# AugmentariumLab/VolumeRenderer

Hardware: AMD Instinct MI355X
Metric: Mvoxels/s kd-tree compress+decode (higher is better)
Workload: dtype u8; 1 GPU; 2048x2048x1920 uint8 volume per GPU as 960 bricks of 256x256x128, rm_volume, tolerance 1, maxEpochs 2, VolumeKdtree build + levelCut

## Files before the change

### volumerenderer_amd/csrc/kd_encode.hip

```cpp
#include "brickset.h"
#include <math.h>
#include <stdio.h>
#include <stdlib.h>
#include <string.h>

namespace vr {

#define FILL_NODES_PER_BLOCK 1024
#define EMIT_RANKS_PER_BLOCK 256

template <bool FROM_VOXELS>
__global__ void __launch_bounds__(256)
k_pyramid(Geom g, int dLeaf, int L, const uint8_t *__restrict__ vox, const uint8_t *__restrict__ inMin,
          const uint8_t *__restrict__ inMax, int64_t inStride, uint8_t *__restrict__ temp, int64_t heapStride,
          uint8_t *__restrict__ tempRange, uint8_t *__restrict__ outMin, uint8_t *__restrict__ outMax,
          int64_t outStride, const uint32_t *__restrict__ srcIdx)
{
    __shared__ uint8_t smn[2][1024], smx[2][1024];
    const int brick = blockIdx.y;
    const uint32_t n = 1u << L;
    const uint32_t base = blockIdx.x << L;
    uint8_t *T = temp + (int64_t)brick * heapStride;
    uint8_t *TR = tempRange ? tempRange + (int64_t)brick * heapStride : nullptr;
    for (uint32_t i = threadIdx.x; i < n; i += blockDim.x) {
// ... 210 lines not shown
    }
    const vr_s16x2 mn3 = pk_pair_min(pk_u(mn2[0]), pk_u(mn2[1])), mx3 = pk_pair_max(pk_u(mx2[0]), pk_u(mx2[1]));
    {
        const int64_t o = ((int64_t)1 << (D - 3)) + (base >> 3) + t * 2;
        const uint32_t m3 = pk_mid(mn3, mx3), h3 = pk_half_range(mn3, mx3);
        *(uint16_t *)(T + o) = (uint16_t)((m3 & 0xFFu) | ((m3 >> 8) & 0xFF00u));
        if (TR) *(uint16_t *)(TR + o) = (uint16_t)((h3 & 0xFFu) | ((h3 >> 8) & 0xFF00u));
    }
    int mn = min((int)mn3.x, (int)mn3.y), mx = max((int)mx3.x, (int)mx3.y);
    {
        const int64_t o = ((int64_t)1 << (D - 4)) + (base >> 4) + t;
        T[o] = (uint8_t)((mn + mx) >> 1);
        if (TR) TR[o] = (uint8_t)((mx - mn) >> 1);
    }
    uint32_t p = (uint32_t)mn | ((uint32_t)(255 - mx) << 16);
#pragma unroll
    for (int k = 1; k <= 6; ++k) {
        uint32_t q;
        if (k == 1) q = dpp_u32<0x101, 0xf>(p, p);
        else if (k == 2) q = dpp_u32<0x102, 0xf>(p, p);
        else if (k == 3) q = dpp_u32<0x104, 0xf>(p, p);
        else if (k == 4) q = dpp_u32<0x108, 0xf>(p, p);
        else q = (uint32_t)__shfl_down((int)p, 1 << (k - 1));
        p = pk_u(__builtin_elementwise_min(pk_s(p), pk_s(q)));
        if ((lane & ((1 << k) - 1)) == 0) {
            const int a = (int)(p & 0xFFFFu), b = 255 - (int)(p >> 16);
            const int64_t o = ((int64_t)1 << (D - 4 - k)) + (base >> (4 + k)) + (t >> k);
            T[o] = (uint8_t)((a + b) >> 1);
            if (TR) TR[o] = (uint8_t)((b - a) >> 1);
        }
    }
    if (lane == 0) mm[t >> 6] = p;
}

__device__ __forceinline__ void pyr12_box_root(const uint32_t *mm, int D, uint32_t base, int brick, uint8_t *__restrict__ T,
                                               uint8_t *__restrict__ TR, uint8_t *__restrict__ outMin, uint8_t *__restrict__ outMax,
                                               int64_t outStride, uint8_t *__restrict__ blockFlag, uint8_t *__restrict__ blockFlagR)
{
    {
        int a[2], b[2];
#pragma unroll
        for (int h = 0; h < 2; ++h) {
            const uint32_t u = pk_u(__builtin_elementwise_min(pk_s(mm[2 * h]), pk_s(mm[2 * h + 1])));
            a[h] = (int)(u & 0xFFFFu); b[h] = 255 - (int)(u >> 16);
            const int64_t o = ((int64_t)1 << (D - 11)) + (base >> 11) + h;
            T[o] = (uint8_t)((a[h] + b[h]) >> 1);
            if (TR) TR[o] = (uint8_t)((b[h] - a[h]) >> 1);
        }
        const int ra = min(a[0], a[1]), rbm = max(b[0], b[1]);
        const int64_t o = ((int64_t)1 << (D - 12)) + (base >> 12);
        T[o] = (uint8_t)((ra + rbm) >> 1);
        if (TR) TR[o] = (uint8_t)((rbm - ra) >> 1);
        outMin[(int64_t)brick * outStride + (base >> 12)] = (uint8_t)ra;
        outMax[(int64_t)brick * outStride + (base >> 12)] = (uint8_t)rbm;
        if (blockFlag) blockFlag[(int64_t)brick * ((int64_t)1 << (D - 12)) + (base >> 12)] = ra == rbm ? 1u : 0u;
        if (blockFlagR) blockFlagR[(int64_t)brick * ((int64_t)1 << (D - 12)) + (base >> 12)] = ra == rbm ? 1u : 0u;
    }
}

#ifndef VR_PYR_LINES_IMAGE_BOXES
#define VR_PYR_LINES_IMAGE_BOXES 8
#endif
#define PYR_LINES_IMAGE_STRIDE (4096 + 16)

__global__ void __launch_bounds__(256)
k_pyramid12_lines(Geom g, Pyr12Geom pg, const uint8_t *__restrict__ vox, uint8_t *__restrict__ temp, int64_t heapStride,
                  uint8_t *__restrict__ tempRange, uint8_t *__restrict__ outMin, uint8_t *__restrict__ outMax,
                  int64_t outStride, uint8_t *__restrict__ blockFlag, uint8_t *__restrict__ blockFlagR)
{
    constexpr int NB = VR_PYR_LINES_IMAGE_BOXES;
    static_assert(NB == 8 || NB == 4, "images per round");
    __shared__ __attribute__((aligned(16))) uint8_t leaf[NB * PYR_LINES_IMAGE_STRIDE];
    __shared__ uint32_t boxConst[4][8];
    __shared__ uint32_t waveMM[8][4];
    const int brick = blockIdx.y, D = g.D;
    const int t = threadIdx.x, lane = t & 63, c = t & 7;
    const uint32_t gid = blockIdx.x;
    const int lgx = pg.lnbx - 3;
    const int gx = (int)((gid & ((1u << lgx) - 1u)) << 7), by = (int)(((gid >> lgx) & ((1u << pg.lnby) - 1u)) << pg.ay),
              bz = (int)((gid >> (lgx + pg.lnby)) << pg.az);
    const int ymask = (1 << pg.ay) - 1;
    const uint8_t *src = vox + (int64_t)brick * g.voxels + (gx + c * 16) + (int64_t)g.X * (by + (int64_t)g.Y * bz);
    uint4 v[8];
#pragma unroll
    for (int k = 0; k < 8; ++k) {
        const int row = (t >> 3) + 32 * k;
        v[k] = *(const uint4 *)(src + (int64_t)g.X * ((row & ymask) + (int64_t)g.Y * (row >> pg.ay)));
    }
    const uint32_t *sp = pg.spread;
    const uint32_t rowBase = sp[g.X + by] | sp[g.X + g.Y + bz];
    uint8_t *T = temp + (int64_t)brick * heapStride;
    uint8_t *TR = tempRange ? tempRange + (int64_t)brick * heapStride : nullptr;
    uint32_t constMask = 0u;
    bool myConst = false;
    if (blockFlag) {
        const uint32_t v0 = __builtin_amdgcn_perm(0, v[0].x, 0u);
        uint32_t diff = 0u;
#pragma unroll
        for (int k = 0; k < 8; ++k) diff |= (v[k].x ^ v0) | (v[k].y ^ v0) | (v[k].z ^ v0) | (v[k].w ^ v0);
        const uint32_t ref = (uint32_t)__shfl((int)v0, c);
        const uint64_t same = __ballot(diff == 0u && v0 == ref), boxLanes = 0x0101010101010101ull << c;
        if (lane < 8) boxConst[t >> 6][lane] = (same & boxLanes) == boxLanes ? v0 : 0x100u;
        __syncthreads();
        const uint32_t c0 = boxConst[0][c];
        myConst = c0 != 0x100u && boxConst[1][c] == c0 && boxConst[2][c] == c0 && boxConst[3][c] == c0;
        constMask = (uint32_t)__ballot(myConst) & 0xFFu;
        if (constMask) {
            const int b = t >> 5, j = t & 31;
            const uint32_t cv = (uint32_t)__shfl((int)c0, b);
            if ((constMask >> b) & 1u) {
                const uint32_t base = sp[gx + 16 * b] | rowBase;
#pragma unroll
                for (int m = 0; m < 4; ++m)
                    pyr12_const_slot(j + 32 * m, cv, D, base, brick, T, TR, outMin, outMax, outStride, blockFlag, blockFlagR);
            }
            if (constMask == 0xFFu) return;
        }
    }
    const uint32_t rlo = sp[g.X + ((t >> 3) & ymask)] | sp[g.X + g.Y + ((t >> 3) >> pg.ay)];
    for (int h = 0; h < 8 / NB; ++h) {
        if (h) __syncthreads();
        if (!myConst && c / NB == h) {
            uint8_t *img = leaf + (c % NB) * PYR_LINES_IMAGE_STRIDE;
#pragma unroll
            for (int k = 0; k < 8; ++k) {
                const uint32_t r0 = rlo | sp[g.X + ((32 * k) & ymask)] | sp[g.X + g.Y + ((32 * k) >> pg.ay)];
                const uint32_t vw[4] = {v[k].x, v[k].y, v[k].z, v[k].w};
#pragma unroll
                for (int i = 0; i < 16; ++i) img[r0 | pg.sx[i]] = (uint8_t)(vw[i >> 2] >> ((i & 3) * 8));
            }
        }
        __syncthreads();
#pragma unroll 1
        for (int b = h * NB; b < (h + 1) * NB; ++b)
            if (!((constMask >> b) & 1u))
                pyr12_reduce_box(leaf + (b % NB) * PYR_LINES_IMAGE_STRIDE, D, sp[gx + 16 * b] | rowBase, t, T, TR, waveMM[b]);
    }
    __syncthreads();
    if (t < 8 && !((constMask >> t) & 1u))
        pyr12_box_root(waveMM[t], D, sp[gx + 16 * t] | rowBase, brick, T, TR, outMin, outMax, outStride, blockFlag, blockFlagR);
}

struct ReconBufs { uint8_t *b[3]; };

struct SkipBlocks {
    uint8_t *flag;
    int64_t nBlk;
    int Dm2;
};
__device__ __forceinline__ bool skip_block(const SkipBlocks &sk, int brick, int d, uint32_t node)
{
    return sk.flag && d > sk.Dm2 && (sk.flag[(int64_t)brick * sk.nBlk + (node >> (10 + d - sk.Dm2))] & 2u) != 0u;
}

__device__ inline int phys_buf(const Ctrl &c, int role) { return role == 0 ? c.ra : c.rb; }

__global__ void k_ctrl_init(Ctrl *ctrls, const uint8_t *rootMin, const uint8_t *rootMax, int64_t mmStride)
{
    Ctrl &c = ctrls[blockIdx.x];
    if (threadIdx.x) return;
    c.constBrick = 0; c.constVal = 0; c.zeroRun = 0;
    if (rootMin) {
        const int mn = rootMin[(int64_t)blockIdx.x * mmStride], mx = rootMax[(int64_t)blockIdx.x * mmStride];
        c.constBrick = mn == mx ? 1 : 0;
        c.constVal = mn;
    }
    c.currentDistance = c.currentError = c.currentDF = c.currentStepSize = 0.0;
    c.previousDistance = c.previousError = c.previousDF = c.previousStepSize = 0.0;
    c.errMinus = c.errPlus = 0;
    c.statL1 = 0;
    c.numActive = 0;
    c.epoch = 0; c.active = 0; c.fillThisEpoch = 0;
    c.cur = 0; c.prev = 1; c.pendingEqual = 0;
    c.par = 0; c.ra = 1; c.rb = 2;
    c.altValid = 0; c.altSel = 0; c.altDist = 0;
    c.numReverts = 0; c.maxErrBefore = 0; c.maxErrAfter = 0;
    c.estS = 0; c.estC = 0; c.estTbase = 0; c.estFallbacks = 0; c.estSeg = 0; c.estDone = 0; c.emitOverflow = 0;
    for (int i = 0; i < VR_MAX_DEPTH + 8; ++i) c.distanceMap[i] = 0;
}

#define EST_SEG 1024
#define EST_CAND 8
#define EST_ROUNDS 5
#define EST_HEAD 4096

#define est_at(ci, seg) (((int64_t)(ci) * summStride + (int64_t)(seg)) * 4)

__device__ __forceinline__ uint32_t wave_incl_scan_u32(uint32_t v, int lane)
{
    (void)lane;
    return wave_incl_scan_add_dpp(v);
}

__device__ __forceinline__ uint32_t lane_u32(uint32_t v, int l) { return (uint32_t)__builtin_amdgcn_readlane((int)v, l); }
__device__ __forceinline__ unsigned long long lane_u64(unsigned long long v, int l)
{
    return (unsigned long long)lane_u32((uint32_t)v, l) | ((unsigned long long)lane_u32((uint32_t)(v >> 32), l) << 32);
}

#define EST_STAGE_NODES 4096
__device__ inline void est_exact_chain(const uint8_t *__restrict__ T, const uint8_t *__restrict__ P, int d, uint32_t lo,
                                       uint32_t hi, unsigned long long &S, uint32_t &C, int lane, const SkipBlocks &sk, int brick,
                                       uint8_t *stage = nullptr)
{
    const uint32_t len = hi - lo;
    const bool staged = stage && d > 0 && len >= 64u && len <= (uint32_t)EST_STAGE_NODES && (len & 63u) == 0u && (lo & 31u) == 0u;
    const uint8_t *sT = stage, *sP = stage + EST_STAGE_NODES;
    if (staged) {
        for (uint32_t i = (uint32_t)lane * 16u; i < len; i += 1024u) *(uint4 *)(stage + i) = *(const uint4 *)(T + lo + i);
        for (uint32_t i = (uint32_t)lane * 16u; i < len / 2u; i += 1024u) *(uint4 *)(stage + EST_STAGE_NODES + i) = *(const uint4 *)(P + (lo >> 1) + i);
    }
    const bool sk0 = skip_block(sk, brick, d, lo);
    int tn = 0, pn = 0;
    if (staged) { tn = sT[lane]; pn = sP[lane >> 1]; }
    else { tn = (!sk0 && lo + lane < hi) ? T[lo + lane] : 0; pn = (!sk0 && lo + lane < hi && d > 0) ? P[(lo + lane) >> 1] : 0; }
    bool skipThis = sk0;
    for (uint32_t base = lo; base < hi; base += 64) {
        uint32_t i = base + lane;
        bool valid = i < hi;
        const int t = tn, p = pn;
        const bool skipped = skipThis;
        {
            const uint32_t i2 = i + 64;
            skipThis = base + 64 < hi && skip_block(sk, brick, d, base + 64);
            if (staged) {
                const uint32_t j2 = i2 - lo;
                tn = j2 < len ? sT[j2] : 0;
                pn = j2 < len ? sP[j2 >> 1] : 0;
            } else {
                tn = (!skipThis && i2 < hi) ? T[i2] : 0;
                pn = (!skipThis && i2 < hi && d > 0) ? P[i2 >> 1] : 0;
            }
        }
        if (skipped) continue;
        int pd = p > t ? p - t : t - p;
        bool forced = (t > p && 2 * t - p > 255) || (t < p && 2 * t < p);
        bool cand = valid && pd > 0;
        bool dec = cand && (forced || S < (unsigned long long)pd * (2ull * C + 1ull));
        unsigned long long mask = __ballot(dec);
        for (int it = 0; it < 65; ++it) {
            uint32_t cpre = __popcll(mask & ((1ull << lane) - 1ull));
            uint32_t v = dec ? (uint32_t)pd : 0u;
            uint32_t spre = wave_incl_scan_u32(v, lane) - v;
            bool nd = cand && (forced || (S + spre) < (unsigned long long)pd * (2ull * (C + cpre) + 1ull));
            unsigned long long nmask = __ballot(nd);
            dec = nd;
            if (nmask == mask) break;
            mask = nmask;
        }
        S += (uint32_t)__builtin_amdgcn_readlane((int)wave_incl_scan_add_dpp(dec ? (uint32_t)pd : 0u), 63);
        C += __popcll(mask);
    }
}

__device__ inline int est_window_base(long long T, int nc)
{
    long long b = T - (nc <= 4 ? 1 : 2);
    if (b < 0) b = 0;
    if (b > 256 - nc) b = 256 - nc;
    return (int)b;
}

__device__ inline void est_finish(Ctrl &c, unsigned long long S, uint32_t C, int maxEpochs)
{
    c.currentDistance = C > 0 ? round((double)S / (double)C) : 0.0;
    c.previousDistance = 0.0;
    c.previousStepSize = 255.0;
    c.previousError = 65025.0;
    c.epoch = 0;
    c.active = maxEpochs > 0 ? 1 : 0;
    c.fillThisEpoch = c.active;
    c.errMinus = c.errPlus = 0;
    c.cur = 0; c.prev = 1; c.pendingEqual = 0;
}

__global__ void __launch_bounds__(64)
k_est_head(int d, int maxEpochs, Ctrl *ctrls, const uint8_t *__restrict__ temp, int64_t heapStride, ReconBufs rb,
           int64_t leafStride, SkipBlocks sk)
{
    const int brick = blockIdx.x, lane = threadIdx.x;
    Ctrl &c = ctrls[brick];
    if (c.constBrick) return;
    const uint8_t *T = temp + (int64_t)brick * heapStride + ((int64_t)1 << d);
    const uint8_t *P = rb.b[c.par] + (int64_t)brick * leafStride;
    const uint32_t n = 1u << d;
    unsigned long long S = 0;
    uint32_t C = 0;
    __shared__ __attribute__((aligned(16))) uint8_t stage[EST_STAGE_NODES + EST_STAGE_NODES / 2];
    est_exact_chain(T, P, d, 0, n < EST_HEAD ? n : EST_HEAD, S, C, lane, sk, brick, stage);
    if (lane == 0) {
        if (n <= EST_HEAD) est_finish(c, S, C, maxEpochs);
        else {
            c.estS = S; c.estC = C;
            c.estSeg = EST_HEAD / EST_SEG;
            c.estDone = 0;
            c.estTbase = est_window_base((long long)(S / (2ull * C + 1ull)), 4);
        }
    }
}

__device__ __forceinline__ uint32_t seg_incl_scan_add_dpp(uint32_t v)
{
    v = row_incl_scan_add_dpp(v);
    return v + dpp_u32<0x142, 0xa>(0, v);
}
__device__ __forceinline__ int seg_max_i32_dpp(int v)
// ... 200 lines not shown
    uint32_t seg = (uint32_t)c.estSeg;
    int fallbacks = 0;
    uint32_t preSeg = 0xFFFFFFFFu;
    long long preCi = -1;
    uint4 pre[4];
#pragma unroll
    for (int j = 0; j < 4; ++j) pre[j] = make_uint4(0, 0, 0x80000000u, 0x7FFFFFFFu);
    const auto fetch = [&](long long ci_, uint32_t seg_, uint4 (&r)[4]) {
        const uint32_t k0 = seg_ + 4u * (uint32_t)lane;
#pragma unroll
        for (int j = 0; j < 4; ++j) {
            r[j] = make_uint4(0, 0, 0x80000000u, 0x7FFFFFFFu);
            if (k0 + (uint32_t)j < nseg) r[j] = *(const uint4 *)(sm + est_at((int)ci_, k0 + (uint32_t)j));
        }
    };
    while (seg < nseg) {
        const long long ci = Tc - Tbase;
        if (ci < 0 || ci >= nc || (budget >= 0 && !lastRound && fallbacks > budget)) {
            if (!lastRound) {
                if (lane == 0) {
                    c.estS = S; c.estC = C; c.estSeg = (int)seg;
                    c.estTbase = est_window_base(Tc, ncNext);
                    c.estFallbacks += fallbacks;
                }
                return;
            }
            est_exact_chain(T, P, d, seg * EST_SEG, n, S, C, lane, sk, brick);
            fallbacks += (int)(nseg - seg);
            break;
        }
        uint4 r[4];
        if (preSeg == seg && preCi == ci) {
#pragma unroll
            for (int j = 0; j < 4; ++j) r[j] = pre[j];
        } else fetch(ci, seg, r);
        preSeg = seg + 256u; preCi = ci;
        fetch(ci, preSeg, pre);
        const uint32_t k0 = seg + 4u * (uint32_t)lane;
        const uint32_t ssL = r[0].x + r[1].x + r[2].x + r[3].x, scL = r[0].y + r[1].y + r[2].y + r[3].y;
        const uint32_t si = wave_incl_scan_u32(ssL, lane), sci = wave_incl_scan_u32(scL, lane);
        uint32_t eS = si - ssL, eC = sci - scL;
        int failJ = 4;
        uint32_t fS = 0, fC = 0;
#pragma unroll
        for (int j = 0; j < 4; ++j) {
            const long long S0 = (long long)S + (long long)eS;
            const long long q = 2ll * ((long long)C + (long long)eC) + 1ll;
            const bool ok = k0 + (uint32_t)j >= nseg || (S0 - Tc * q >= (long long)(int)r[j].z && S0 - (Tc + 1) * q < (long long)(int)r[j].w);
            if (!ok && failJ == 4) { failJ = j; fS = eS; fC = eC; }
            eS += r[j].x; eC += r[j].y;
        }
        const unsigned long long bad = __ballot(failJ < 4);
        if (bad == 0ull) {
            S += lane_u32(si, 63);
            C += lane_u32(sci, 63);
            seg += 256u;
            continue;
        }
        const int f = __ffsll((long long)bad) - 1;
        S += lane_u32(fS, f);
        C += lane_u32(fC, f);
        seg += 4u * (uint32_t)f + lane_u32((uint32_t)failJ, f);
        est_exact_chain(T, P, d, seg * EST_SEG, (seg + 1) * EST_SEG, S, C, lane, sk, brick, stage);
        Tc = (long long)(S / (2ull * C + 1ull));
        seg += 1;
        ++fallbacks;
    }
    if (lane == 0) { est_finish(c, S, C, maxEpochs); c.estFallbacks += fallbacks; c.estDone = 1; }
}

__device__ inline unsigned long long block_sum_u64(unsigned long long v, unsigned long long *sh)
{
    for (int o = 32; o > 0; o >>= 1) v += __shfl_xor(v, o);
    const int w = threadIdx.x >> 6;
    if ((threadIdx.x & 63) == 0) sh[w] = v;
    __syncthreads();
    unsigned long long r = 0;
    if (threadIdx.x == 0) for (int i = 0; i < (int)(blockDim.x >> 6); ++i) r += sh[i];
    __syncthreads();
    return r;
}

__global__ void __launch_bounds__(256)
k_fill(int d, Ctrl *ctrls, const uint8_t *__restrict__ temp, uint8_t *__restrict__ codes, int64_t heapStride,
       int64_t codeStride, ReconBufs rb, int64_t leafStride, unsigned long long *__restrict__ blockErr, int64_t nErrBlk)
{
    __shared__ unsigned long long sh[4];
    const int brick = blockIdx.y;
    Ctrl &c = ctrls[brick];
    if (c.constBrick || !c.fillThisEpoch) return;
    const uint32_t n = 1u << d;
    const uint8_t *T = temp + (int64_t)brick * heapStride + ((int64_t)1 << d);
    uint8_t *Cb = codes + (int64_t)brick * codeStride;
    const uint8_t *P = rb.b[c.par] + (int64_t)brick * leafStride;
    uint8_t *R = rb.b[phys_buf(c, c.cur)] + (int64_t)brick * leafStride;
    const int dist = (int)(uint8_t)c.currentDistance;
    const int distM = (int)(uint8_t)fmax(0.0, c.currentDistance - 1.0);
    const int distP = (int)(uint8_t)fmin(255.0, c.currentDistance + 1.0);
    unsigned long long e0 = 0, em = 0, ep = 0;
    const uint32_t i0 = (blockIdx.x * 256u + threadIdx.x) * 4u;
    uint32_t pk = 0;
#pragma unroll
    for (int k = 0; k < 4; ++k) {
        uint32_t i = i0 + k;
        if (i < n) {
            int t = T[i];
            int p = d > 0 ? P[i >> 1] : 0;
            Enc e = encode_node(t, p, dist);
            pk |= (uint32_t)e.code << (2 * k);
            R[i] = (uint8_t)e.recon;
            e0 += (unsigned)(e.err * e.err);
            int a = encode_node(t, p, distM).err, b = encode_node(t, p, distP).err;
            em += (unsigned)(a * a);
            ep += (unsigned)(b * b);
        }
    }
    if (i0 < n) {
        if (d >= 2) Cb[(((int64_t)1 << d) + i0) >> 2] = (uint8_t)pk;
        else if (d == 0) Cb[0] = (uint8_t)((Cb[0] & ~0x0Cu) | (pk << 2));
        else Cb[0] = (uint8_t)((Cb[0] & 0x0Fu) | ((pk & 0xFu) << 4));
    }
    e0 = block_sum_u64(e0, sh);
    em = block_sum_u64(em, sh);
    ep = block_sum_u64(ep, sh);
    if (threadIdx.x == 0) {
        blockErr[(int64_t)brick * nErrBlk + blockIdx.x] = e0;
        if (em) atomicAdd(&c.errMinus, em);
        if (ep) atomicAdd(&c.errPlus, ep);
    }
}

__device__ __forceinline__ unsigned long long wave_sum_u64(unsigned long long v)
{
    for (int o = 32; o > 0; o >>= 1) v += __shfl_xor(v, o);
    return v;
}

__device__ __forceinline__ void leaf_pair_encode(uint32_t tword, int tsel, uint32_t pword, int psel, uint32_t dR2, uint32_t dC2,
                                                 vr_s16x2 &dl, uint32_t &codes2)
{
    const EncPair c = enc_pair(tword, tsel, pword, psel);
    const vr_s16x2 x = enc_pair_x(c, dR2), nx = (vr_s16x2)(0) - x, ax = __builtin_elementwise_max(x, nx);
    uint32_t take = pk_u((ax - c.pd) >> 15);
    const uint32_t stepD = (c.up & pk_u(nx)) | (~c.up & pk_u(x));
    dl = pk_s((take & stepD) | (~take & pk_u(c.T2 - c.P2)));
    if (dC2 != dR2) {
        const vr_s16x2 xc = enc_pair_x(c, dC2);
        take = pk_u((pk_abs(xc) - c.pd) >> 15);
    }
    codes2 = take & pk_u(pk_s(c.up) + pk_s(0x00020002u));
}

#define FILL_ITERS 8
template <bool STORE>
__global__ void __launch_bounds__(256)
k_fill16(int d, int maxEpochs, Ctrl *ctrls, const uint8_t *__restrict__ temp, uint8_t *__restrict__ codes, int64_t heapStride,
         int64_t codeStride, ReconBufs rb, int64_t leafStride, unsigned long long *__restrict__ blockErr, int64_t nErrBlk,
         SkipBlocks sk, int64_t errPlane, int iters)
{
    __shared__ unsigned long long shm[4], shp[4];
    const int brick = blockIdx.y;
    Ctrl &c = ctrls[brick];
    const int cConst = c.constBrick, cFill = c.fillThisEpoch, cPar = c.par, cCur = c.cur, cRa = c.ra, cRb = c.rb, cEpoch = c.epoch;
    const double cDist = c.currentDistance;
    if (cConst || !cFill) return;
    if (!STORE && c.altSel) return;
    const uint8_t *T = temp + (int64_t)brick * heapStride + ((int64_t)1 << d);
    uint8_t *Cd = codes + (int64_t)brick * codeStride + ((int64_t)1 << (d - 2));
    const int rPhys = cCur == 0 ? cRa : cRb;
    const uint8_t *P = (cPar == 0 ? rb.b[0] : (cPar == 1 ? rb.b[1] : rb.b[2])) + (int64_t)brick * leafStride;
    uint8_t *R = (rPhys == 0 ? rb.b[0] : (rPhys == 1 ? rb.b[1] : rb.b[2])) + (int64_t)brick * leafStride;
    const int dist = (int)(uint8_t)cDist;
    const int distM = (int)(uint8_t)fmax(0.0, cDist - 1.0);
    const int distP = (int)(uint8_t)fmin(255.0, cDist + 1.0);
    const bool needDF = cEpoch + 1 < maxEpochs;
    const uint32_t d2 = (uint32_t)dist * 0x10001u, dm2 = (uint32_t)distM * 0x10001u, dp2 = (uint32_t)distP * 0x10001u;
    const int w = threadIdx.x >> 6;
    const uint32_t nchunk = (uint32_t)(((size_t)1 << d) >> 12);
    uint32_t chunk = blockIdx.x * (uint32_t)iters;
    const uint32_t chunkEnd = chunk + (uint32_t)iters < nchunk ? chunk + (uint32_t)iters : nchunk;
    unsigned long long accM = 0, accP = 0;
    bool skippedN = skip_block(sk, brick, d, (chunk * 4u + (uint32_t)w) << 10);
    uint4 tvN = make_uint4(0, 0, 0, 0);
    uint2 pvN = make_uint2(0, 0);
    if (!skippedN) { const size_t i0 = ((size_t)chunk * 256u + threadIdx.x) * 16u; tvN = ld16(T + i0); pvN = ld8(P + (i0 >> 1)); }
    for (; chunk < chunkEnd; ++chunk) {
    const size_t i0 = ((size_t)chunk * 256u + threadIdx.x) * 16u;
    const bool skipped = skippedN;
    const uint4 tv = tvN;
    const uint2 pv = pvN;
    if (chunk + 1 < chunkEnd) {
        skippedN = skip_block(sk, brick, d, ((chunk + 1u) * 4u + (uint32_t)w) << 10);
        tvN = make_uint4(0, 0, 0, 0); pvN = make_uint2(0, 0);
        if (!skippedN) { const size_t i1 = i0 + 4096u; tvN = ld16(T + i1); pvN = ld8(P + (i1 >> 1)); }
    }
    const uint32_t tw[4] = {tv.x, tv.y, tv.z, tv.w}, pw[2] = {pv.x, pv.y};
    uint32_t e0 = 0, em = 0, ep = 0, wa = 0, wb = 0, rw[4] = {tw[0], tw[1], tw[2], tw[3]}, rprev = 0;
    const uint32_t differs = (tw[0] ^ __builtin_amdgcn_perm(0, pw[0], 0x01010000u)) | (tw[1] ^ __builtin_amdgcn_perm(0, pw[0], 0x03030202u)) |
                             (tw[2] ^ __builtin_amdgcn_perm(0, pw[1], 0x01010000u)) | (tw[3] ^ __builtin_amdgcn_perm(0, pw[1], 0x03030202u));
    const bool busy = !skipped && __ballot(differs != 0u) != 0ull;
    if (sk.flag && d == sk.Dm2 && !busy && (threadIdx.x & 63) == 0) {
        uint8_t *f = sk.flag + (int64_t)brick * sk.nBlk + (size_t)chunk * 4 + w;
        if (*f & 1u) *f = 3u;
    }
    const auto pair = [&](const int j) {
        const EncPair c = enc_pair(tw[j >> 1], j & 1, pw[j >> 2], j & 3);
        const vr_s16x2 x = enc_pair_x(c, d2), ax = pk_abs(x);
        e0 = pk_sumsq(__builtin_elementwise_min(c.pd, ax), e0);
        if (STORE) {
        const uint32_t take = pk_u((ax - c.pd) >> 15);
        const uint32_t code2 = take & pk_u(pk_s(c.up) + pk_s(0x00020002u));
        if (j < 4) wa |= code2 << (4 * j); else wb |= code2 << (4 * (j - 4));
        const vr_s16x2 r = pk_mad(x, pk_mad(pk_s(c.up), pk_s(0xFFFEFFFEu), pk_s(0xFFFFFFFFu)), c.T2);
        const uint32_t rec = (take & pk_u(r)) | (~take & pk_u(c.P2));
        if (j & 1) rw[j >> 1] = __builtin_amdgcn_perm(rec, rprev, 0x06040200u); else rprev = rec;
        }
        if (needDF) {
            em = pk_sumsq(enc_pair_err(c, dm2), em);
            ep = pk_sumsq(enc_pair_err(c, dp2), ep);
        }
    };
    bool uniform = false;
    if (busy) {
        const uint32_t t0 = __builtin_amdgcn_perm(0, tw[0], 0u), p0 = __builtin_amdgcn_perm(0, pw[0], 0u);
        const uint32_t mixed = (tw[0] ^ t0) | (tw[1] ^ t0) | (tw[2] ^ t0) | (tw[3] ^ t0) | (pw[0] ^ p0) | (pw[1] ^ p0);
        uniform = __ballot(mixed != 0u) == 0ull;
    }
    if (uniform) {
        pair(0);
        e0 *= 8u; em *= 8u; ep *= 8u;
        if (STORE) {
            wa *= 0x1111u; wb = wa;
            rw[0] = rw[1] = rw[2] = rw[3] = __builtin_amdgcn_perm(0, rprev, 0u);
        }
    } else if (busy)
#pragma unroll
        for (int j = 0; j < 8; ++j) pair(j);
    const uint32_t cpk = ((wa | (wa >> 14)) & 0xFFFFu) | ((wb | (wb >> 14)) << 16);
    if (!skipped && STORE) {
        st4(Cd + (i0 >> 2), cpk);
        st16(R + i0, make_uint4(rw[0], rw[1], rw[2], rw[3]));
    }
    unsigned long long s0 = 0, sm = 0, sp = 0;
    if (busy) {
        s0 = (uint32_t)__builtin_amdgcn_readlane((int)wave_incl_scan_add_dpp(e0), 63);
        sm = (uint32_t)__builtin_amdgcn_readlane((int)wave_incl_scan_add_dpp(em), 63);
        sp = (uint32_t)__builtin_amdgcn_readlane((int)wave_incl_scan_add_dpp(ep), 63);
    }
    if ((threadIdx.x & 63) == 0) {
        blockErr[(int64_t)brick * nErrBlk + (size_t)chunk * 4 + w] = s0;
        if (!STORE && needDF) {
            blockErr[errPlane + (int64_t)brick * nErrBlk + (size_t)chunk * 4 + w] = sm;
            blockErr[2 * errPlane + (int64_t)brick * nErrBlk + (size_t)chunk * 4 + w] = sp;
        }
    }
    accM += sm; accP += sp;
    }
    if ((threadIdx.x & 63) == 0) { shm[w] = accM; shp[w] = accP; }
    __syncthreads();
    if (threadIdx.x == 0) {
        const unsigned long long tm = shm[0] + shm[1] + shm[2] + shm[3], tp = shp[0] + shp[1] + shp[2] + shp[3];
        if (tm) atomicAdd(&c.errMinus, tm);
        if (tp) atomicAdd(&c.errPlus, tp);
    }
}

__device__ __forceinline__ double next_pow2_above(double s)
{
    int ex;
    frexp(s, &ex);
    return ldexp(1.0, ex);
}

__device__ inline double ctl_walk_block(double s, const uint8_t *__restrict__ T, const uint8_t *__restrict__ P, int d,
                                        int dist, uint32_t lo, uint32_t hi, int lane)
{
    int tn = lo + lane < hi ? T[lo + lane] : 0, pn = (lo + lane < hi && d > 0) ? P[(lo + lane) >> 1] : 0;
    for (uint32_t base = lo; base < hi; base += 64) {
        uint32_t i = base + lane;
        uint32_t e = 0;
        const int t = tn, p = pn;
        {
            const uint32_t i2 = i + 64;
            tn = i2 < hi ? T[i2] : 0;
            pn = (i2 < hi && d > 0) ? P[i2 >> 1] : 0;
        }
        if (i < hi) {
            int er = encode_node(t, p, dist).err;
            e = (uint32_t)(er * er);
        }
        const uint32_t incl = wave_incl_scan_u32(e, lane);
        const uint32_t total = lane_u32(incl, 63);
        uint32_t consumed = 0;
        int start = 0;
        while (true) {
            bool ok = true;
            if (lane >= start && s != 0.0) ok = (s + (double)(incl - consumed)) < next_pow2_above(s);
            const unsigned long long bad = ~__ballot(ok);
            if (bad == 0ull) { s = s + (double)(total - consumed); break; }
            const int f = __ffsll((long long)bad) - 1;
            const uint32_t exclF = lane_u32(incl - e, f), eF = lane_u32(e, f);
            s = s + (double)(exclF - consumed);
            s = s + (double)eF;
            consumed = exclF + eF;
            start = f + 1;
        }
    }
    return s;
}

__device__ inline double ctl_walk_block16(double s, const uint8_t *__restrict__ T, const uint8_t *__restrict__ P, int dist,
                                          uint32_t lo, int lane)
{
    const uint4 tv = *(const uint4 *)(T + lo + lane * 16);
    const uint2 pv = *(const uint2 *)(P + (lo >> 1) + lane * 8);
    const uint32_t tw[4] = {tv.x, tv.y, tv.z, tv.w}, pw[2] = {pv.x, pv.y};
    const uint32_t d2 = (uint32_t)dist * 0x10001u;
    uint32_t e[16], pre[16];
    uint32_t run = 0;
#pragma unroll
    for (int j = 0; j < 8; ++j) {
        const EncPair c = enc_pair(tw[j >> 1], j & 1, pw[j >> 2], j & 3);
        const vr_s16x2 er = enc_pair_err(c, d2);
        e[2 * j] = (uint32_t)((int)er.x * (int)er.x);
        e[2 * j + 1] = (uint32_t)((int)er.y * (int)er.y);
        run += e[2 * j]; pre[2 * j] = run;
        run += e[2 * j + 1]; pre[2 * j + 1] = run;
    }
    const uint32_t inclL = wave_incl_scan_add_dpp(run);
    const uint32_t baseL = inclL - run, total = (uint32_t)__builtin_amdgcn_readlane((int)inclL, 63);
    uint32_t consumed = 0;
    int startPos = 0;
    while (true) {
        int fail = 16;
        if (s != 0.0) {
            const double bound = next_pow2_above(s);
#pragma unroll
            for (int k = 15; k >= 0; --k)
                if (lane * 16 + k >= startPos && !((s + (double)(baseL + pre[k] - consumed)) < bound)) fail = k;
        }
        const unsigned long long bad = __ballot(fail < 16);
        if (bad == 0ull) { s = s + (double)(total - consumed); break; }
        const int f = __ffsll((long long)bad) - 1;
        const int kF = __builtin_amdgcn_readlane(fail, f);
        uint32_t eF = 0, gF = 0;
#pragma unroll
        for (int k = 0; k < 16; ++k) if (k == kF) { eF = e[k]; gF = baseL + pre[k]; }
        eF = (uint32_t)__builtin_amdgcn_readlane((int)eF, f);
        gF = (uint32_t)__builtin_amdgcn_readlane((int)gF, f);
        s = s + (double)(gF - eF - consumed);
        s = s + (double)eF;
        consumed = gF;
        startPos = f * 16 + kF + 1;
    }
    return s;
}

#define CTL_STAGE_BLOCKS 8192
__device__ inline double ctl_partials64(double s, const unsigned long long *__restrict__ be, const uint32_t *stg, uint32_t base, uint32_t nblk,
                                        const uint8_t *__restrict__ T, const uint8_t *__restrict__ P, int d, int dist,
                                        uint32_t n, int lane)
{
    const unsigned long long e2 = base + lane < nblk ? (stg ? (unsigned long long)stg[base + lane] : be[base + lane]) : 0ull;
    const unsigned long long incl = (unsigned long long)wave_incl_scan_add_dpp((uint32_t)(e2 & 0xFFFFFFull)) +
                                    ((unsigned long long)wave_incl_scan_add_dpp((uint32_t)(e2 >> 24)) << 24);
    const unsigned long long total = lane_u64(incl, 63);
    unsigned long long consumed = 0;
    int start = 0;
    while (true) {
        bool ok = true;
        const bool sInt = (s == floor(s)) && (s + (double)(total - consumed)) < 9007199254740992.0;
        if (lane >= start && !sInt) ok = (s + (double)(incl - consumed)) < next_pow2_above(s);
        const unsigned long long bad = ~__ballot(ok);
        if (bad == 0ull) { s = s + (double)(total - consumed); break; }
        const int f = __ffsll((long long)bad) - 1;
        const unsigned long long exclF = lane_u64(incl - e2, f), inclF = lane_u64(incl, f);
        s = s + (double)(exclF - consumed);
        uint32_t lo = (base + f) * FILL_NODES_PER_BLOCK, hi = lo + FILL_NODES_PER_BLOCK;
        if (hi > n) hi = n;
        s = (hi - lo == 1024u && d > 0) ? ctl_walk_block16(s, T, P, dist, lo, lane) : ctl_walk_block(s, T, P, d, dist, lo, hi, lane);
        consumed = inclF;
        start = f + 1;
    }
    return s;
}

__global__ void __launch_bounds__(64)
k_control(int d, int maxEpochs, int guarded, Ctrl *ctrls, const uint8_t *__restrict__ temp, int64_t heapStride,
          ReconBufs rb, int64_t leafStride, const unsigned long long *__restrict__ blockErr, int64_t nErrBlk, int64_t errPlane,
          int leaflessLeaf)
{
    const int brick = blockIdx.x, lane = threadIdx.x;
    __shared__ __attribute__((aligned(16))) uint32_t ctlStage[CTL_STAGE_BLOCKS];
    Ctrl &c = ctrls[brick];
    if (c.constBrick) return;
    const uint32_t n = 1u << d;
    const bool ending = c.active && c.fillThisEpoch;
    double s = c.currentError;
    if (ending) {
        const uint8_t *T = temp + (int64_t)brick * heapStride + ((int64_t)1 << d);
        const uint8_t *P = rb.b[c.par] + (int64_t)brick * leafStride;
        const int dist = (int)(uint8_t)c.currentDistance;
        const uint32_t nblk = (n + FILL_NODES_PER_BLOCK - 1) / FILL_NODES_PER_BLOCK;
        const unsigned long long *be = blockErr + (int64_t)c.altSel * errPlane + (int64_t)brick * nErrBlk;
        const uint32_t nchunk = (nblk + 63u) >> 6;
        const uint32_t *stg = nullptr;
        if (nblk >= 256u && nblk <= (uint32_t)CTL_STAGE_BLOCKS && (nblk & 255u) == 0u) {
            for (uint32_t i = (uint32_t)lane * 4u; i < nblk; i += 256u) {
                const uint4 a = *(const uint4 *)(be + i), b = *(const uint4 *)(be + i + 2);
                *(uint4 *)(ctlStage + i) = make_uint4(a.x, a.z, b.x, b.z);
// ... 1904 lines not shown
```

Baseline: 302,100 Mvoxels/s.

## Batch skip-flag reads per wave and iterate only live chunks in k_fill16

k_fill16 now loads all skip/const flag bytes for a workgroup's chunks up front, one per lane, and turns them into ballot masks. The chunk loop then visits only non-skipped chunks with a two-deep ping-pong prefetch. Error outputs and const-flag updates are written once per lane after the loop instead of by lane 0 on every iteration. This removes serialized per-chunk flag loads and branch overhead on skipped chunks, at the cost of more register pressure and more complex control flow.

```diff
diff --git a/volumerenderer_amd/csrc/kd_encode.hip b/volumerenderer_amd/csrc/kd_encode.hip
--- a/volumerenderer_amd/csrc/kd_encode.hip
+++ b/volumerenderer_amd/csrc/kd_encode.hip
@@ -386,6 +386,10 @@
 {
     return sk.flag && d > sk.Dm2 && (sk.flag[(int64_t)brick * sk.nBlk + (node >> (10 + d - sk.Dm2))] & 2u) != 0u;
 }
+
+#ifndef VR_FLAGS_BATCHED
+#define VR_FLAGS_BATCHED 1
+#endif
 
 __device__ inline int phys_buf(const Ctrl &c, int role) { return role == 0 ? c.ra : c.rb; }
 
@@ -892,6 +896,7 @@
 }
 
 #define FILL_ITERS 8
+static_assert(FILL_ITERS < 32, "k_fill16 keeps a workgroup's chunks as the bits of a 32-bit mask and the lanes of a wave");
 template <bool STORE>
 __global__ void __launch_bounds__(256)
 k_fill16(int d, int maxEpochs, Ctrl *ctrls, const uint8_t *__restrict__ temp, uint8_t *__restrict__ codes, int64_t heapStride,
@@ -899,7 +904,14 @@
          SkipBlocks sk, int64_t errPlane, int iters)
 {
     __shared__ unsigned long long shm[4], shp[4];
-    const int brick = blockIdx.y;
+    const int brick = blockIdx.y, lane = threadIdx.x & 63;
+#if VR_FLAGS_BATCHED
+    uint32_t flagByte = 0;
+    if (sk.flag && d >= sk.Dm2) {
+        const uint32_t nch = (uint32_t)(((size_t)1 << d) >> 12), cj = blockIdx.x * (uint32_t)iters + (uint32_t)lane;
+        if (lane < iters && cj < nch) flagByte = sk.flag[(int64_t)brick * sk.nBlk + ((cj * 4u + (threadIdx.x >> 6)) >> (d - sk.Dm2))];
+    }
+#endif
     Ctrl &c = ctrls[brick];
     const int cConst = c.constBrick, cFill = c.fillThisEpoch, cPar = c.par, cCur = c.cur, cRa = c.ra, cRb = c.rb, cEpoch = c.epoch;
     const double cDist = c.currentDistance;
@@ -920,29 +932,18 @@
     uint32_t chunk = blockIdx.x * (uint32_t)iters;
     const uint32_t chunkEnd = chunk + (uint32_t)iters < nchunk ? chunk + (uint32_t)iters : nchunk;
     unsigned long long accM = 0, accP = 0;
-    bool skippedN = skip_block(sk, brick, d, (chunk * 4u + (uint32_t)w) << 10);
-    uint4 tvN = make_uint4(0, 0, 0, 0);
-    uint2 pvN = make_uint2(0, 0);
-    if (!skippedN) { const size_t i0 = ((size_t)chunk * 256u + threadIdx.x) * 16u; tvN = ld16(T + i0); pvN = ld8(P + (i0 >> 1)); }
-    for (; chunk < chunkEnd; ++chunk) {
-    const size_t i0 = ((size_t)chunk * 256u + threadIdx.x) * 16u;
-    const bool skipped = skippedN;
-    const uint4 tv = tvN;
-    const uint2 pv = pvN;
-    if (chunk + 1 < chunkEnd) {
-        skippedN = skip_block(sk, brick, d, ((chunk + 1u) * 4u + (uint32_t)w) << 10);
-        tvN = make_uint4(0, 0, 0, 0); pvN = make_uint2(0, 0);
-        if (!skippedN) { const size_t i1 = i0 + 4096u; tvN = ld16(T + i1); pvN = ld8(P + (i1 >> 1)); }
-    }
+#if VR_FLAGS_BATCHED
+    const uint32_t skipMask = d > sk.Dm2 ? (uint32_t)__ballot((flagByte & 2u) != 0u) : 0u;
+    const uint32_t constMask = d == sk.Dm2 ? (uint32_t)__ballot((flagByte & 1u) != 0u) : 0u;
+#endif
+    const auto eval = [&](const uint4 tv, const uint2 pv, const bool skipped, uint32_t &cpk, uint32_t (&rw)[4], uint32_t &s0,
+                          uint32_t &sm, uint32_t &sp) -> bool {
     const uint32_t tw[4] = {tv.x, tv.y, tv.z, tv.w}, pw[2] = {pv.x, pv.y};
-    uint32_t e0 = 0, em = 0, ep = 0, wa = 0, wb = 0, rw[4] = {tw[0], tw[1], tw[2], tw[3]}, rprev = 0;
+    uint32_t e0 = 0, em = 0, ep = 0, wa = 0, wb = 0, rprev = 0;
+    rw[0] = tw[0]; rw[1] = tw[1]; rw[2] = tw[2]; rw[3] = tw[3];
     const uint32_t differs = (tw[0] ^ __builtin_amdgcn_perm(0, pw[0], 0x01010000u)) | (tw[1] ^ __builtin_amdgcn_perm(0, pw[0], 0x03030202u)) |
                              (tw[2] ^ __builtin_amdgcn_perm(0, pw[1], 0x01010000u)) | (tw[3] ^ __builtin_amdgcn_perm(0, pw[1], 0x03030202u));
     const bool busy = !skipped && __ballot(differs != 0u) != 0ull;
-    if (sk.flag && d == sk.Dm2 && !busy && (threadIdx.x & 63) == 0) {
-        uint8_t *f = sk.flag + (int64_t)brick * sk.nBlk + (size_t)chunk * 4 + w;
-        if (*f & 1u) *f = 3u;
-    }
     const auto pair = [&](const int j) {
         const EncPair c = enc_pair(tw[j >> 1], j & 1, pw[j >> 2], j & 3);
         const vr_s16x2 x = enc_pair_x(c, d2), ax = pk_abs(x);
@@ -976,26 +977,97 @@
     } else if (busy)
 #pragma unroll
         for (int j = 0; j < 8; ++j) pair(j);
-    const uint32_t cpk = ((wa | (wa >> 14)) & 0xFFFFu) | ((wb | (wb >> 14)) << 16);
-    if (!skipped && STORE) {
-        st4(Cd + (i0 >> 2), cpk);
-        st16(R + i0, make_uint4(rw[0], rw[1], rw[2], rw[3]));
-    }
-    unsigned long long s0 = 0, sm = 0, sp = 0;
+    cpk = ((wa | (wa >> 14)) & 0xFFFFu) | ((wb | (wb >> 14)) << 16);
+    s0 = sm = sp = 0;
     if (busy) {
         s0 = (uint32_t)__builtin_amdgcn_readlane((int)wave_incl_scan_add_dpp(e0), 63);
         sm = (uint32_t)__builtin_amdgcn_readlane((int)wave_incl_scan_add_dpp(em), 63);
         sp = (uint32_t)__builtin_amdgcn_readlane((int)wave_incl_scan_add_dpp(ep), 63);
     }
-    if ((threadIdx.x & 63) == 0) {
-        blockErr[(int64_t)brick * nErrBlk + (size_t)chunk * 4 + w] = s0;
+    return busy;
+    };
+#if VR_FLAGS_BATCHED
+    const uint32_t cnt = chunkEnd - chunk, liveMask = ((1u << cnt) - 1u) & ~skipMask;
+    uint32_t errS = 0, errM = 0, errP = 0, exactMask = 0;
+    if (liveMask) {
+        uint32_t m = liveMask;
+        const size_t idle = ((size_t)(chunk + (31u - (uint32_t)__builtin_clz(liveMask))) * 256u + (size_t)(w << 6)) * 16u;
+        int kA, kB;
+        uint4 tA, tB;
+        uint2 pA, pB;
+        const auto next = [&](int &k, uint4 &tv, uint2 &pv) {
+            k = m ? __builtin_ctz(m) : -1;
+            m &= m - 1u;
+            const size_t i = k >= 0 ? ((size_t)(chunk + (uint32_t)k) * 256u + threadIdx.x) * 16u : idle;
+            tv = ld16(T + i); pv = ld8(P + (i >> 1));
+        };
+        const auto phase = [&](int &k, uint4 &tv, uint2 &pv) {
+            const int kc = k;
+            const size_t i0 = ((size_t)(chunk + (uint32_t)kc) * 256u + threadIdx.x) * 16u;
+            uint32_t cpk, rw[4], s0, sm, sp;
+            const bool busy = eval(tv, pv, false, cpk, rw, s0, sm, sp);
+            if (STORE) {
+                st4(Cd + (i0 >> 2), cpk);
+                st16(R + i0, make_uint4(rw[0], rw[1], rw[2], rw[3]));
+            }
+            next(k, tv, pv);
+            if (lane == kc) { errS = s0; errM = sm; errP = sp; }
+            accM += sm; accP += sp;
+            if (!busy) exactMask |= 1u << kc;
+        };
+        next(kA, tA, pA);
+        next(kB, tB, pB);
+        phase(kA, tA, pA);
+        while (kB >= 0) {
+            phase(kB, tB, pB);
+            if (kA < 0) break;
+            phase(kA, tA, pA);
+        }
+    }
+    if ((uint32_t)lane < cnt) {
+        const int64_t at = (int64_t)brick * nErrBlk + (size_t)(chunk + (uint32_t)lane) * 4 + w;
+        blockErr[at] = errS;
         if (!STORE && needDF) {
-            blockErr[errPlane + (int64_t)brick * nErrBlk + (size_t)chunk * 4 + w] = sm;
-            blockErr[2 * errPlane + (int64_t)brick * nErrBlk + (size_t)chunk * 4 + w] = sp;
-        }
-    }
-    accM += sm; accP += sp;
-    }
+            blockErr[errPlane + at] = errM;
+            blockErr[2 * errPlane + at] = errP;
+        }
+        if (((exactMask & constMask) >> lane) & 1u) sk.flag[(int64_t)brick * sk.nBlk + (size_t)(chunk + (uint32_t)lane) * 4 + w] = 3u;
+    }
+#else
+    bool skippedN = skip_block(sk, brick, d, (chunk * 4u + (uint32_t)w) << 10);
+    uint4 tvN = make_uint4(0, 0, 0, 0);
+    uint2 pvN = make_uint2(0, 0);
+    if (!skippedN) { const size_t i0 = ((size_t)chunk * 256u + threadIdx.x) * 16u; tvN = ld16(T + i0); pvN = ld8(P + (i0 >> 1)); }
+    for (; chunk < chunkEnd; ++chunk) {
+        const size_t i0 = ((size_t)chunk * 256u + threadIdx.x) * 16u;
+        const bool skipped = skippedN;
+        const uint4 tv = tvN;
+        const uint2 pv = pvN;
+        if (chunk + 1 < chunkEnd) {
+            skippedN = skip_block(sk, brick, d, ((chunk + 1u) * 4u + (uint32_t)w) << 10);
+            tvN = make_uint4(0, 0, 0, 0); pvN = make_uint2(0, 0);
+            if (!skippedN) { const size_t i1 = i0 + 4096u; tvN = ld16(T + i1); pvN = ld8(P + (i1 >> 1)); }
+        }
+        uint32_t cpk, rw[4], s0, sm, sp;
+        const bool busy = eval(tv, pv, skipped, cpk, rw, s0, sm, sp);
+        if (sk.flag && d == sk.Dm2 && !busy && lane == 0) {
+            uint8_t *f = sk.flag + (int64_t)brick * sk.nBlk + (size_t)chunk * 4 + w;
+            if (*f & 1u) *f = 3u;
+        }
+        if (!skipped && STORE) {
+            st4(Cd + (i0 >> 2), cpk);
+            st16(R + i0, make_uint4(rw[0], rw[1], rw[2], rw[3]));
+        }
+        if (lane == 0) {
+            blockErr[(int64_t)brick * nErrBlk + (size_t)chunk * 4 + w] = s0;
+            if (!STORE && needDF) {
+                blockErr[errPlane + (int64_t)brick * nErrBlk + (size_t)chunk * 4 + w] = sm;
+                blockErr[2 * errPlane + (int64_t)brick * nErrBlk + (size_t)chunk * 4 + w] = sp;
+            }
+        }
+        accM += sm; accP += sp;
+    }
+#endif
     if ((threadIdx.x & 63) == 0) { shm[w] = accM; shp[w] = accP; }
     __syncthreads();
     if (threadIdx.x == 0) {
```

Measured after the change: 311,200 Mvoxels/s, median of 6. +3.0%, better.
